# facebookresearch/co-tracker

Hardware: AMD Instinct MI355X
Metric: tracked-point-frames/sec (N*T/s) (higher is better)
Workload: dtype f32 (Linear layers as split-half f16 MFMA x3, f32 accumulate); 1 GPU; 512x512 T=120 N=6400 cotracker3 online-weights sliding window S=16 (BASELINE.json configs[2]); points_per_gpu=6400, frames=120, iters=6, window_len=16, offline=False, precision=f16x3, weights=seeded synthetic (no checkpoints offline)

## Files before the change

co-tracker_amd/csrc/api.hip:

```cpp
#include "ctk_common.h"
#include "ctk_profile.h"
#include "gemm_params.h"
#include "ctk_options.h"
#include <cstdlib>
#include <mutex>
#include <new>

int ctk_launch_corr_volume(const ctk_window_args* a, int n0, int ncount, float* out, long level_stride, int ld,
                           hipStream_t s, bool groups = false);
int ctk_launch_pyramid_split(const float* fmap, long pixels, void* out, int version, hipStream_t s);
int ctk_launch_corr_volume_sh(const ctk_window_args* a, const void* const* fm_sh, int n0, int ncount, void* out,
                              long level_stride_halves, int version, hipStream_t s, bool groups = false);
int ctk_launch_virtual_init(const float* vt, int S, float* dst, int B, hipStream_t s);
int ctk_launch_layernorm2(const float* x, void* y, long R, const float* gamma, const float* beta, float eps, void* y2, float eps2,
                          int out_split, hipStream_t s);
int ctk_launch_heads(const float* tokens, const float* hw, const float* hb, int S, int N, float* delta, float* coords,
                     float* vis, float* conf, hipStream_t s);
int ctk_launch_assemble(const ctk_window_args* a, void* x, int x_split, int ld, int base, hipStream_t s);
int ctk_launch_assemble_batch(const CtkBatchState& st, int B, int S, int N, float scale_x, float scale_y, void* x, int x_split,
                              int ld, int base, hipStream_t s);
int ctk_launch_heads_batch(const float* tokens, const float* hw, const float* hb, const CtkBatchState& st, int B, int S, int N,
                           hipStream_t s);

namespace {

inline size_t align256(size_t x) { return (x + 255) & ~(size_t)255; }

#define CTK_TRY(expr)        \
  do {                       \
    int rc__ = (expr);       \
    if (rc__) return rc__;   \
  } while (0)

class EventRing {
 public:
  int next(hipEvent_t* out) {
    int dev = 0;
    hipError_t rc = hipGetDevice(&dev);
    if (rc != hipSuccess) return (int)rc;
    if (dev < 0 || dev >= kMaxDev) return CTK_E_STATE;
    std::lock_guard<std::mutex> g(m_);
    PerDev& d = d_[dev];
    if (!d.ready) {
      for (int i = 0; i < kN; ++i) {
        rc = hipEventCreateWithFlags(&d.ev[i], hipEventDisableTiming);
        if (rc != hipSuccess) {
          for (int j = 0; j < i; ++j) (void)hipEventDestroy(d.ev[j]);
          return (int)rc;
        }
      }
      d.ready = true;
    }
    *out = d.ev[d.i];
    d.i = (d.i + 1) % kN;
    return CTK_OK;
  }

 private:
  static constexpr int kN = 256, kMaxDev = 64;
  struct PerDev {
    hipEvent_t ev[kN];
    int i = 0;
    bool ready = false;
  };
  std::mutex m_;
  PerDev d_[kMaxDev];
};
EventRing g_events;

int stream_follow(hipStream_t from, hipStream_t to) {
  hipEvent_t e;
  CTK_TRY(g_events.next(&e));
  hipError_t rc = hipEventRecord(e, from);
  if (rc != hipSuccess) return (int)rc;
  rc = hipStreamWaitEvent(to, e, 0);
  return rc == hipSuccess ? CTK_OK : (int)rc;
}

int overlap_mode() { return ctk_opt(CTK_OPT_OVERLAP); }

struct JoinGuard {
  hipStream_t main, aux;
  bool open = false;
  int fork() {
    const int rc = stream_follow(main, aux);
    open = rc == CTK_OK;
    return rc;
  }
  int join() {
    open = false;
    return stream_follow(aux, main);
  }
  ~JoinGuard() {
    if (open) (void)stream_follow(aux, main);
  }
};

struct WRef {
  const float* w;
  const void* p;
};

struct Linear {
  ctk_gemm_args g{};
  Linear(const float* x, long M, WRef W, int N, int K, float* y, const float* bias) {
    g.A = x; g.lda = K; g.M = (int)M; g.W = W.w; g.Wp = W.p; g.ldw = K; g.N = N; g.K = K; g.C = y; g.ldc = N; g.bias = bias;
    g.act = CTK_ACT_NONE; g.batch = 1;
  }
  Linear& act(int a) { g.act = a; return *this; }
  Linear& ldy(long ld) { g.ldc = ld; return *this; }
  Linear& add(const float* resid) { g.resid = resid; return *this; }
  Linear& bias_rows(const float* rows, int period) { g.bias_rows = rows; g.bias_period = period; return *this; }
  Linear& k_valid(int k) { g.k_valid = k; return *this; }
  Linear& batched(int n, long x_bs, long y_bs) { g.batch = n; g.a_bs = x_bs; g.c_bs = y_bs; return *this; }
  Linear& sh(bool in, bool out) { g.a_split = in; g.c_split = out; return *this; }
  int run(hipStream_t s) {
    if (g.resid) g.ldr = g.ldc;
    if (g.a_split) { g.lda *= 2; g.a_bs *= 2; }
    if (g.c_split) { g.ldc *= 2; g.c_bs *= 2; }
    return ctk_gemm(&g, s);
  }
};

bool split_mode(const ctk_model_weights* w) { return w->in_p != nullptr; }
bool folded(const ctk_model_weights* w) { return !w->corr_fc2_w && !w->corr_fc2_p; }

struct UfWs {
  float* tokens;
  float* xn;
  float* xn2;
  float* qkv;
  float* att;
  float* hid;
  float* partial;
  size_t bytes;
};

int v2p_splits(int N) {
  int s = (N + 1023) / 1024;
  if (s < 1) s = 1;
  if (s > 32) s = 32;
  return s;
}

UfWs carve_uf(int S, int N, void* base, int B = 1) {
  const size_t R = (size_t)B * (N + CTK_VIRT) * S;
  UfWs w;
  char* p = static_cast<char*>(base);
  size_t off = 0;
  auto take = [&](size_t nfloat) {
    float* r = reinterpret_cast<float*>(p + off);
    off += align256(nfloat * sizeof(float));
    return r;
  };
  w.tokens = take(R * CTK_HID);
  w.xn = take(R * CTK_HID);
  w.xn2 = take((size_t)B * N * S * CTK_HID);
  w.qkv = take(R * 3 * CTK_HID);
  w.att = take(R * CTK_HID);
  w.hid = take(R * CTK_MLP);
  w.partial = take((size_t)v2p_splits(N) * B * S * CTK_HEADS * CTK_VIRT * (CTK_HEAD_DIM + 2));
  w.bytes = off;
  return w;
}

int attn(const float* q, long q_ld, long q_bs, long q_is, const float* k, const float* v, long kv_ld, long kv_bs,
         long kv_is, float* out, long o_bs, long o_is, int nbatch, int n1, int n2, int splits, float* partial,
         hipStream_t s, bool o_split, const uint8_t* key_mask = nullptr, const uint8_t* query_mask = nullptr,
         const ctk_attn_batch2* b2 = nullptr) {
  ctk_attn_args a;
  a.key_mask = key_mask; a.query_mask = query_mask;
  a.q = q; a.q_ld = q_ld; a.q_bs = q_bs; a.q_is = q_is;
  a.k = k; a.v = v; a.kv_ld = kv_ld; a.kv_bs = kv_bs; a.kv_is = kv_is;
  a.out = out; a.o_ld = o_split ? 2 * CTK_HID : CTK_HID; a.o_bs = o_bs; a.o_is = o_is; a.o_split = o_split;
  a.nbatch = nbatch; a.n1 = n1; a.n2 = n2; a.splits = splits; a.partial = partial;
  return ctk_attention_ex(&a, b2, s);
}

int mlp_block(const UfWs& ws, long r0, long R, const ctk_block_weights& b, hipStream_t s, bool sp) {
  float* tok = ws.tokens + r0 * CTK_HID;
  float* xn = ws.xn + r0 * CTK_HID;
  float* hid = ws.hid + r0 * CTK_MLP;
  CTK_TRY(ctk_layernorm(tok, xn, R, nullptr, nullptr, 1e-6f, sp, s));
  CTK_TRY(Linear(xn, R, {b.w1, b.w1_p}, CTK_MLP, CTK_HID, hid, b.b1).act(CTK_ACT_GELU_TANH).sh(sp, sp).run(s));
  CTK_TRY(Linear(hid, R, {b.w2, b.w2_p}, CTK_HID, CTK_MLP, tok, b.b2).add(tok).sh(sp, false).run(s));
  return CTK_OK;
}

struct FormerRef {
  int depth;
  const ctk_block_weights* time_blocks;
  const ctk_block_weights* virtual2point;
  const ctk_block_weights* virtual_self;
  const ctk_block_weights* point2virtual;
  const float* virtual_tokens;
  const uint8_t* point_mask;
  bool split;
  hipStream_t aux;
  bool space_attn = true;
  int B = 1;
};

FormerRef former_of(const ctk_model_weights* w) {
  return FormerRef{CTK_DEPTH, w->time_blocks, w->virtual2point, w->virtual_self, w->point2virtual, w->virtual_tokens, nullptr,
                   w->in_p != nullptr, nullptr};
}

int run_transformer(int S, int N, const FormerRef& fr, const UfWs& ws, hipStream_t s) {
  const FormerRef* w = &fr;
  const bool sp = fr.split;
  const int B = fr.B;
  const long P = (long)B * N * S;
  const long V = (long)B * CTK_VIRT * S;
  const long PS = (long)N * S, VS = (long)CTK_VIRT * S;
  const bool joint = B > 1;
  if (joint && fr.point_mask) return CTK_E_STATE;
  const ctk_attn_batch2 v2p_b{S, 0, VS, PS, VS, 0, 0};
  const ctk_attn_batch2 vself_b{S, 0, VS, VS, VS, 0, 0};
  const ctk_attn_batch2 p2v_b{S, 0, PS, VS, PS, 0, 0};
  const long R = P + V;
  const long QL = 3 * CTK_HID;
  struct Rows { float *tok, *xn, *att, *q, *k, *v; };
  auto rows_from = [&](long r) {
    return Rows{ws.tokens + r * CTK_HID, ws.xn + r * CTK_HID, ws.att + r * CTK_HID, ws.qkv + r * QL, ws.qkv + r * QL + CTK_HID, ws.qkv + r * QL + 2 * CTK_HID};
  };
  const Rows pt = rows_from(0), vt = rows_from(P);
  auto to_q = [&](const ctk_block_weights& b, const float* xn, long rows, const Rows& q, hipStream_t st) {
    return Linear(xn, rows, {b.wq, b.wq_p}, CTK_HID, CTK_HID, q.q, b.bq).ldy(QL).sh(sp, false).run(st);
  };
  auto to_kv = [&](const ctk_block_weights& b, const Rows& kv, long rows) {
    return Linear(kv.xn, rows, {b.wkv, b.wkv_p}, 2 * CTK_HID, CTK_HID, kv.k, b.bkv).ldy(QL).sh(sp, false).run(s);
  };
  auto to_out = [&](const ctk_block_weights& b, const Rows& q, long rows) {
    return Linear(q.att, rows, {b.wo, b.wo_p}, CTK_HID, CTK_HID, q.tok, b.bo).add(q.tok).sh(sp, false).run(s);
  };
  CTK_TRY(ctk_launch_virtual_init(w->virtual_tokens, S, vt.tok, B, s));

  for (int i = 0; i < fr.depth; ++i) {
    {
      const ctk_block_weights& b = w->time_blocks[i];
      CTK_TRY(ctk_layernorm(pt.tok, pt.xn, R, nullptr, nullptr, 1e-6f, sp, s));
      CTK_TRY(to_q(b, pt.xn, R, pt, s));
      CTK_TRY(to_kv(b, pt, R));
      CTK_TRY(attn(pt.q, QL, S, 1, pt.k, pt.v, QL, S, 1, pt.att, S, 1, B * (N + CTK_VIRT), S, S, 1, nullptr, s, sp));
      CTK_TRY(to_out(b, pt, R));
      CTK_TRY(mlp_block(ws, 0, R, b, s, sp));
    }
    if (!fr.space_attn) continue;
    const bool side_q = fr.aux != nullptr && (overlap_mode() & 2) != 0;
    JoinGuard side{s, fr.aux};
    if (side_q) {
      CTK_TRY(side.fork());
      CTK_TRY(ctk_layernorm(pt.tok, ws.xn2, P, nullptr, nullptr, 1e-6f, sp, fr.aux));
      CTK_TRY(to_q(w->point2virtual[i], ws.xn2, P, pt, fr.aux));
    }
    {
      const ctk_block_weights& b = w->virtual2point[i];
      CTK_TRY(ctk_layernorm(vt.tok, vt.xn, V, nullptr, nullptr, 1e-6f, sp, s));
      if (!side_q) CTK_TRY(ctk_launch_layernorm2(pt.tok, pt.xn, P, b.ctx_gamma, b.ctx_beta, 1e-5f, ws.xn2, 1e-6f, sp, s));
      else CTK_TRY(ctk_layernorm(pt.tok, pt.xn, P, b.ctx_gamma, b.ctx_beta, 1e-5f, sp, s));
      CTK_TRY(to_q(b, vt.xn, V, vt, s));
      CTK_TRY(to_kv(b, pt, P));
      CTK_TRY(attn(vt.q, QL, 1, S, pt.k, pt.v, QL, 1, S, vt.att, 1, S, B * S, CTK_VIRT, N,
                   v2p_splits(N), ws.partial, s, sp, fr.point_mask, nullptr, joint ? &v2p_b : nullptr));
      CTK_TRY(to_out(b, vt, V));
      CTK_TRY(mlp_block(ws, P, V, b, s, sp));
    }
    {
      const ctk_block_weights& b = w->virtual_self[i];
      CTK_TRY(ctk_layernorm(vt.tok, vt.xn, V, nullptr, nullptr, 1e-6f, sp, s));
      CTK_TRY(to_q(b, vt.xn, V, vt, s));
      CTK_TRY(to_kv(b, vt, V));
      CTK_TRY(attn(vt.q, QL, 1, S, vt.k, vt.v, QL, 1, S, vt.att, 1, S, B * S,
                   CTK_VIRT, CTK_VIRT, 1, nullptr, s, sp, nullptr, nullptr, joint ? &vself_b : nullptr));
      CTK_TRY(to_out(b, vt, V));
      CTK_TRY(mlp_block(ws, P, V, b, s, sp));
    }
    {
      const ctk_block_weights& b = w->point2virtual[i];
      CTK_TRY(ctk_layernorm(vt.tok, vt.xn, V, b.ctx_gamma, b.ctx_beta, 1e-5f, sp, s));
      if (!side_q) CTK_TRY(to_q(b, ws.xn2, P, pt, s));
      else CTK_TRY(side.join());
      CTK_TRY(to_kv(b, vt, V));
      CTK_TRY(attn(pt.q, QL, 1, S, vt.k, vt.v, QL, 1, S, pt.att, 1, S, B * S, N, CTK_VIRT, 1, nullptr, s, sp,
                   nullptr, fr.point_mask, joint ? &p2v_b : nullptr));
      CTK_TRY(to_out(b, pt, P));
      CTK_TRY(mlp_block(ws, 0, P, b, s, sp));
    }
  }
  return CTK_OK;
}

int check_former(const FormerRef& fr) {
  auto check_block = [&](const ctk_block_weights& b, bool cross) {
    if (!b.bq || !b.bkv || !b.bo || !b.b1 || !b.b2) return CTK_E_NULL;
    if ((!b.wq && !b.wq_p) || (!b.wkv && !b.wkv_p) || (!b.wo && !b.wo_p) || (!b.w1 && !b.w1_p) || (!b.w2 && !b.w2_p)) return CTK_E_NULL;
    if (cross && (!b.ctx_gamma || !b.ctx_beta)) return CTK_E_NULL;
    const bool all_p = b.wq_p && b.wkv_p && b.wo_p && b.w1_p && b.w2_p, any_p = b.wq_p || b.wkv_p || b.wo_p || b.w1_p || b.w2_p;
    return (fr.split ? !all_p : any_p) ? CTK_E_NULL : CTK_OK;
  };
  for (int i = 0; i < fr.depth; ++i) {
    CTK_TRY(check_block(fr.time_blocks[i], false));
    CTK_TRY(check_block(fr.virtual2point[i], true));
    CTK_TRY(check_block(fr.virtual_self[i], false));
    CTK_TRY(check_block(fr.point2virtual[i], true));
  }
  return CTK_OK;
}

int check_weights(const ctk_model_weights* w, bool window = false) {
  if (!w) return CTK_E_NULL;
  if ((!w->in_w && !w->in_p) || !w->in_bias_t || !w->virtual_tokens || !w->head_w || !w->head_b) return CTK_E_NULL;
  if (folded(w)) {
    if (!window || (!w->corr_fc1_w && !w->corr_fc1_p) || !w->corr_fc1_b) return CTK_E_NULL;
    if (split_mode(w) != (w->corr_fc1_p != nullptr)) return CTK_E_NULL;
  } else if (split_mode(w) != (w->corr_fc1_p && w->corr_fc2_p)) {
    return CTK_E_NULL;
  }
  return check_former(former_of(w));
}

int input_projection(int S, int N, const float* x, bool x_split, const ctk_model_weights* w, const UfWs& ws, hipStream_t s,
                     bool fold = false) {
  return Linear(x, N * S, {w->in_w, w->in_p}, CTK_HID, fold ? CTK_XF_LD : CTK_X_LD, ws.tokens, nullptr)
      .bias_rows(w->in_bias_t, S).k_valid(fold ? CTK_XF_DIM : CTK_X_DIM).sh(x_split, false).run(s);
}

struct CorrWs {
  float* vol;
  float* h1;
  void* fm_sh[CTK_MAX_BATCH][CTK_LEVELS];
  size_t bytes;
  int chunk;
  int corr_version;
};

int corr_chunk_points(const ctk_window_args* a, int B = 1) {
  const long all = (long)B * a->N;
  long c = a->points_per_chunk > 0 ? a->points_per_chunk : all;
  if (c > all) c = all;
  return (int)c;
}

CorrWs carve_corr(const ctk_window_args* a, void* base, int B = 1, bool shared = false, bool fold = false) {
  CorrWs w;
  w.corr_version = ctk_opt(CTK_OPT_CORR_VERSION);
  w.chunk = corr_chunk_points(a, B);
  const size_t rows = (size_t)w.chunk * a->S;
  char* p = static_cast<char*>(base);
  size_t off = 0;
  w.vol = reinterpret_cast<float*>(p + off);
  off += align256(rows * CTK_LEVELS * CTK_CORR_LD * sizeof(float));
  w.h1 = fold ? nullptr : reinterpret_cast<float*>(p + off);
  if (!fold) off += align256(rows * CTK_LEVELS * CTK_HID * sizeof(float));
  for (int b = 0; b < B; ++b)
    for (int l = 0; l < CTK_LEVELS; ++l) {
      if (shared && b > 0) {
        w.fm_sh[b][l] = w.fm_sh[0][l];
        continue;
      }
      w.fm_sh[b][l] = p + off;
      off += align256((size_t)a->S * (a->H[l] > 0 ? a->H[l] : 0) * (a->W[l] > 0 ? a->W[l] : 0) * CTK_C * sizeof(float));
    }
  w.bytes = off;
  return w;
}

int prepare_pyramid_sh(const ctk_window_args* videos, const CorrWs& ws, hipStream_t s, int B = 1) {
  for (int b = 0; b < B; ++b) {
    const ctk_window_args* a = videos + b;
    for (int l = 0; l < CTK_LEVELS; ++l) {
      if (!a->fmaps[l]) return CTK_E_NULL;
      if (a->H[l] <= 0 || a->W[l] <= 0) return CTK_E_SHAPE;
      CTK_TRY(ctk_launch_pyramid_split(a->fmaps[l], (long)a->S * a->H[l] * a->W[l], ws.fm_sh[b][l], ws.corr_version, s));
    }
  }
  return CTK_OK;
}

int run_corr_embed(const ctk_window_args* videos, int B, const ctk_model_weights* w, float* x, bool x_split, const CorrWs& ws,
                   hipStream_t s, bool shared = false, bool fold = false) {
  const ctk_window_args* a = videos;
  const bool sp = split_mode(w);
  if (x_split && !sp) return CTK_E_SHAPE;
  if ((!w->corr_fc1_w && !w->corr_fc1_p) || !w->corr_fc1_b) return CTK_E_NULL;
  if (fold != folded(w) || (!fold && !w->corr_fc2_b)) return CTK_E_NULL;
  hipStream_t aux = B == 1 ? static_cast<hipStream_t>(a->aux_stream) : nullptr;
  const bool pipelined = sp && aux != nullptr && (overlap_mode() & 1) != 0;
  const int NT = B * a->N;
  for (int n0 = 0; n0 < NT; n0 += ws.chunk) {
    const int cnt = (NT - n0 < ws.chunk) ? NT - n0 : ws.chunk;
    const int pieces = pipelined ? ((cnt >= 4096) ? 4 : (cnt >= 1024 ? 2 : 1)) : 1;
    const int per = (cnt + pieces - 1) / pieces;
    JoinGuard pipe{s, aux};
    for (int j = 0; j < pieces; ++j) {
      const int p0 = j * per;
      const int pc = (cnt - p0 < per) ? cnt - p0 : per;
      if (pc <= 0) break;
      const long rows = (long)pc * a->S;
      float* vol = ws.vol + (size_t)p0 * a->S * CTK_LEVELS * CTK_CORR_LD;
      float* h1 = fold ? nullptr : ws.h1 + (size_t)p0 * a->S * CTK_LEVELS * CTK_HID;
      hipStream_t gs = s;
      const int g0 = n0 + p0;
      if (shared && B > 1) {
        if (sp) CTK_TRY(ctk_launch_corr_volume_sh(a, ws.fm_sh[0], g0, pc, vol, rows * CTK_CORR_LD * 2, ws.corr_version, s, true));
        else CTK_TRY(ctk_launch_corr_volume(a, g0, pc, vol, rows * CTK_CORR_LD, CTK_CORR_LD, s, true));
      } else {
        for (int b = g0 / a->N; b < B && b * a->N < g0 + pc; ++b) {
          const int lo = g0 > b * a->N ? g0 : b * a->N;
          const int hi = g0 + pc < (b + 1) * a->N ? g0 + pc : (b + 1) * a->N;
          const int m0 = lo - b * a->N, mc = hi - lo;
          float* vb = vol + (size_t)(lo - g0) * a->S * CTK_CORR_LD;
          if (sp) CTK_TRY(ctk_launch_corr_volume_sh(videos + b, ws.fm_sh[b], m0, mc, vb, rows * CTK_CORR_LD * 2, ws.corr_version, s));
          else CTK_TRY(ctk_launch_corr_volume(videos + b, m0, mc, vb, rows * CTK_CORR_LD, CTK_CORR_LD, s));
        }
      }
      if (pipelined && pieces > 1) {
// ... 453 lines not shown
```

co-tracker_amd/csrc/attention.hip:

```cpp
#include "ctk_common.h"
#include "ctk_options.h"
#include "ctk_profile.h"
#include "gemm_params.h"
#include <cstdlib>

namespace {

constexpr int HD = CTK_HEAD_DIM;
constexpr int KC = 16;
constexpr int MAXB = 8;
constexpr int BPAD = 4;
constexpr float NEG_MAX = -3.402823466e+38f;

struct AttnP {
  const float* q; long q_ld, q_bs, q_is;
  const float* k; const float* v; long kv_ld, kv_bs, kv_is;
  float* out; long o_ld, o_bs, o_is;
  int nbatch, n1, n2;
  int splits, keys_per_split;
  float* partial;
  int o_split;
  int bpw;
  int qtiles;
  float scale;
// ... 820 lines not shown
    }
    if (!more) break;
    job = next;
  }
}

constexpr int TR_LD = 3 * CTK_HID;
constexpr int TR_PITCH = TR_LD + VT_PITCH;
constexpr int TR_CHUNKS = TR_LD / 4;
constexpr int TR_LOADS = 32 * TR_CHUNKS / 512;
static_assert(TR_PITCH % 64 == VT_PITCH && (TR_PITCH * 4) % 16 == 0 && 32 * TR_CHUNKS == 512 * TR_LOADS && TR_CHUNKS % 8 == 0, "pair block layout");
static_assert(16 * TR_CHUNKS == 512 * (TR_LOADS / 2), "a track is a whole number of workgroup loads");
static_assert(32 * TR_PITCH * 4 <= 160 * 1024, "one pair per CU");
constexpr int TR_MIN_ROUNDS = 8;

__global__ __launch_bounds__(512, 1) void attention_time_rows_kernel(AttnP p, int npairs) {
  __shared__ __attribute__((aligned(16))) float blk[32 * TR_PITCH];
  const int tid = threadIdx.x, head = tid >> 6, lane = tid & 63, r32 = lane & 31, half = lane >> 5;
  const int vd0 = r32, vd1 = min(32 + r32, HD - 1);
  const int rb = r32 >> 4, ri = r32 & 15;
  int pair = blockIdx.x;
  if (pair >= npairs) return;
  unsigned char* oimg = reinterpret_cast<unsigned char*>(blk + head * HD);
  const float* qrow = blk + r32 * TR_PITCH + head * HD + half * 8;
  const float* vcol = blk + 2 * CTK_HID + head * HD;

  f32x4 raw[TR_LOADS];
  auto load = [&](const int pr) {
    const float* src = p.q + (long)pr * (32 * TR_LD) + tid * 4;
    const int second = (2 * pr + 1 < p.nbatch) ? (TR_LOADS / 2) * 512 * 4 : 0;
#pragma unroll
    for (int i = 0; i < TR_LOADS / 2; ++i) {
      raw[i] = __builtin_nontemporal_load(reinterpret_cast<const f32x4*>(src + i * 512 * 4));
      raw[i + TR_LOADS / 2] = __builtin_nontemporal_load(reinterpret_cast<const f32x4*>(src + i * 512 * 4 + second));
    }
  };

  load(pair);
  while (true) {
    const int b0 = 2 * pair;
    {
#pragma unroll
      for (int i = 0; i < TR_LOADS / 2; ++i) {
        const int c = 512 * i + tid, row = c / TR_CHUNKS, cc = c - row * TR_CHUNKS;
        float* dst = blk + row * TR_PITCH + cc * 4;
        *reinterpret_cast<f32x4*>(dst) = raw[i];
        *reinterpret_cast<f32x4*>(dst + 16 * TR_PITCH) = raw[i + TR_LOADS / 2];
      }
    }
    const int next = pair + (int)gridDim.x;
    const bool more = next < npairs;
    if (more) load(next);
    __syncthreads();

    f16x8 qh[3], ql[3], kh[3], kl[3], vh[2][2], vl[2][2];
    {
      f32x4 f[6];
#pragma unroll
      for (int j = 0; j < 3; ++j) {
        f[2 * j] = *reinterpret_cast<const f32x4*>(qrow + 16 * j);
        f[2 * j + 1] = *reinterpret_cast<const f32x4*>(qrow + 16 * j + 4);
      }
#pragma unroll
      for (int j = 0; j < 3; ++j) ctk_split8(f[2 * j] * p.scale2, f[2 * j + 1] * p.scale2, qh[j], ql[j]);
#pragma unroll
      for (int j = 0; j < 3; ++j) {
        f[2 * j] = *reinterpret_cast<const f32x4*>(qrow + CTK_HID + 16 * j);
        f[2 * j + 1] = *reinterpret_cast<const f32x4*>(qrow + CTK_HID + 16 * j + 4);
      }
#pragma unroll
      for (int j = 0; j < 3; ++j) ctk_split8(f[2 * j], f[2 * j + 1], kh[j], kl[j]);
    }
    {
      float v0[16], v1[16];
#pragma unroll
      for (int s = 0; s < 2; ++s)
#pragma unroll
        for (int e = 0; e < 8; ++e) {
          const int slot = 16 * s + 8 * (e >> 2) + 4 * half + (e & 3);
          v0[8 * s + e] = vcol[slot * TR_PITCH + vd0];
          v1[8 * s + e] = vcol[slot * TR_PITCH + vd1];
        }
#pragma unroll
      for (int s = 0; s < 2; ++s) {
        ctk_split8(f32x4{v0[8 * s], v0[8 * s + 1], v0[8 * s + 2], v0[8 * s + 3]}, f32x4{v0[8 * s + 4], v0[8 * s + 5], v0[8 * s + 6], v0[8 * s + 7]},
                   vh[0][s], vl[0][s]);
        ctk_split8(f32x4{v1[8 * s], v1[8 * s + 1], v1[8 * s + 2], v1[8 * s + 3]}, f32x4{v1[8 * s + 4], v1[8 * s + 5], v1[8 * s + 6], v1[8 * s + 7]},
                   vh[1][s], vl[1][s]);
      }
    }

    const bool qvalid = b0 + rb < p.nbatch;
    f32x16 sacc;
#pragma unroll
    for (int e = 0; e < 16; ++e) sacc[e] = 0.0f;
#pragma unroll
    for (int j = 0; j < 3; ++j) sacc = ctk_mma3(kh[j], kl[j], qh[j], ql[j], sacc);
    float tmax = -INFINITY;
#pragma unroll
    for (int e = 0; e < 16; ++e) {
      const int slot = 8 * (e >> 2) + 4 * half + (e & 3);
      const bool ok = ((slot >> 4) == rb) && (b0 + (slot >> 4) < p.nbatch);
      sacc[e] = ok ? sacc[e] : -INFINITY;
      tmax = fmaxf(tmax, sacc[e]);
    }
    tmax = fmaxf(tmax, __shfl_xor(tmax, 32, 64));
    const float mnew = (tmax == -INFINITY) ? 0.0f : tmax;
    float l = 0.0f;
#pragma unroll
    for (int e = 0; e < 16; ++e) {
      const float pv = __builtin_amdgcn_exp2f(sacc[e] - mnew);
      l += pv;
      sacc[e] = pv * PSCALE;
    }
    f32x16 oacc[2];
#pragma unroll
    for (int dt = 0; dt < 2; ++dt)
#pragma unroll
      for (int e = 0; e < 16; ++e) oacc[dt][e] = 0.0f;
#pragma unroll
    for (int s = 0; s < 2; ++s) {
      f16x8 ph, pl;
      ctk_split8(f32x4{sacc[8 * s], sacc[8 * s + 1], sacc[8 * s + 2], sacc[8 * s + 3]},
                 f32x4{sacc[8 * s + 4], sacc[8 * s + 5], sacc[8 * s + 6], sacc[8 * s + 7]}, ph, pl);
      oacc[0] = ctk_mma3(vh[0][s], vl[0][s], ph, pl, oacc[0]);
      oacc[1] = ctk_mma3(vh[1][s], vl[1][s], ph, pl, oacc[1]);
    }
    l += __shfl_xor(l, 32, 64);
    const float inv = 1.0f / (l * PSCALE);
    if (p.o_split) {
      attn_store_sh_head<TR_PITCH * 4>(oacc, inv, oimg, lane, head, [&](int row) -> _Float16* {
        const int ob = b0 + (row >> 4), oi = row & 15;
        return ob < p.nbatch ? reinterpret_cast<_Float16*>(p.out) + ((long)ob * p.o_bs + (long)oi * p.o_is) * p.o_ld : nullptr;
      });
    } else if (qvalid) {
      const long orow = ((long)(b0 + rb) * p.o_bs + (long)ri * p.o_is) * p.o_ld;
#pragma unroll
      for (int dt = 0; dt < 2; ++dt)
#pragma unroll
        for (int q = 0; q < 4; ++q) {
          const int d = dt * 32 + q * 8 + half * 4;
          if (d < HD) {
            const f32x4 t = {oacc[dt][4 * q] * inv, oacc[dt][4 * q + 1] * inv, oacc[dt][4 * q + 2] * inv, oacc[dt][4 * q + 3] * inv};
            *reinterpret_cast<f32x4*>(p.out + orow + head * HD + d) = t;
          }
        }
    }
    if (!more) break;
    pair = next;
    __syncthreads();
  }
}

__global__ void attention_merge_kernel(AttnP p) {
  const long i = (long)blockIdx.x * blockDim.x + threadIdx.x;
  const long total = (long)p.nbatch * CTK_HEADS * p.n1 * HD;
  if (i >= total) return;
  const int d = i % HD;
  long r = i / HD;
  const int qi = r % p.n1; r /= p.n1;
  const int head = r % CTK_HEADS;
  const int b = r / CTK_HEADS;
  const long stride = (long)p.nbatch * CTK_HEADS * p.n1 * (HD + 2);
  const float* base = p.partial + (((long)b * CTK_HEADS + head) * p.n1 + qi) * (HD + 2);
  float m = -INFINITY;
  for (int s = 0; s < p.splits; ++s) m = fmaxf(m, base[s * stride]);
  float l = 0.0f, a = 0.0f;
  for (int s = 0; s < p.splits; ++s) {
    const float w = p.log2m ? __builtin_amdgcn_exp2f(base[s * stride] - m) : expf(base[s * stride] - m);
    l += w * base[s * stride + 1];
    a += w * base[s * stride + 2 + d];
  }
  const float o = a / l;
  const long orow = batch_row(b, p.binner, p.o_bs, p.o_obs) + qi * p.o_is;
  if (p.o_split) {
    _Float16* oh = reinterpret_cast<_Float16*>(p.out) + orow * p.o_ld + ctk_sh_col(head * HD + d);
    const _Float16 hi = (_Float16)o;
    oh[0] = hi;
    oh[32] = (_Float16)(o - (float)hi);
  } else {
    p.out[orow * p.o_ld + head * HD + d] = o;
  }
}

int attn_backend() { return ctk_opt(CTK_OPT_ATTENTION_VALU); }

int attn_num_cus() {
  static const int n = [] {
    int dev = 0, cu = 0;
    if (hipGetDevice(&dev) != hipSuccess || hipDeviceGetAttribute(&cu, hipDeviceAttributeMultiprocessorCount, dev) != hipSuccess || cu <= 0) cu = 256;
    return cu;
  }();
  return n;
}

}

extern "C" int ctk_attention(const ctk_attn_args* a, void* stream) { return ctk_attention_ex(a, nullptr, stream); }

extern "C" int ctk_attention_ex(const ctk_attn_args* a, const ctk_attn_batch2* b2, void* stream) {
  if (!a || !a->q || !a->k || !a->v || !a->out) return CTK_E_NULL;
  if (a->nbatch <= 0 || a->n1 <= 0 || a->n2 <= 0) return CTK_E_SHAPE;
  const bool two_level = b2 != nullptr && b2->inner > 0;
  if (two_level && (a->nbatch % b2->inner)) return CTK_E_SHAPE;
  if ((a->q_ld % 4) || (a->kv_ld % 4) || (a->o_ld % 4)) return CTK_E_ALIGN;
  if (!ctk_aligned16(a->q) || !ctk_aligned16(a->k) || !ctk_aligned16(a->v) || !ctk_aligned16(a->out)) return CTK_E_ALIGN;
  AttnP p;
  p.q = a->q; p.q_ld = a->q_ld; p.q_bs = a->q_bs; p.q_is = a->q_is;
  p.k = a->k; p.v = a->v; p.kv_ld = a->kv_ld; p.kv_bs = a->kv_bs; p.kv_is = a->kv_is;
  p.out = static_cast<float*>(a->out); p.o_ld = a->o_ld; p.o_bs = a->o_bs; p.o_is = a->o_is;
  p.o_split = a->o_split;
  if (p.o_split && (a->o_ld % 64)) return CTK_E_ALIGN;
  p.nbatch = a->nbatch; p.n1 = a->n1; p.n2 = a->n2;
  p.splits = a->splits > 1 ? a->splits : 1;
  if (p.splits > 1 && !a->partial) return CTK_E_NULL;
  p.partial = a->partial;
  p.kmask = a->key_mask;
  p.qmask = a->query_mask;
  p.binner = two_level ? b2->inner : a->nbatch;
  p.q_obs = two_level ? b2->q_os : 0; p.kv_obs = two_level ? b2->kv_os : 0; p.o_obs = two_level ? b2->o_os : 0;
  p.km_obs = two_level ? b2->key_mask_os : 0; p.qm_obs = two_level ? b2->query_mask_os : 0;
  p.scale = 0.14433756729740643f;
  p.scale2 = 0.14433756729740643f * 1.4426950408889634f;
  p.log2m = 0;
  hipStream_t s = static_cast<hipStream_t>(stream);
  const double flops = 4.0 * a->nbatch * (double)a->n1 * a->n2 * CTK_HID;
  const double bytes = 4.0 * a->nbatch * ((double)a->n1 * 2 + (double)a->n2 * 2) * CTK_HID;
  const bool mfma = attn_backend() == 0;

  if (mfma && a->n2 == CTK_VIRT) {
    p.splits = 1;
    p.keys_per_split = a->n2;
    p.bpw = 1;
    p.qtiles = 1;
    CtkProfScope ps(a->n1 > CTK_VIRT ? "attention_p2v" : "attention_vself", flops, bytes, s);
    const unsigned gx = (unsigned)((a->n1 + 128 * QT_PER_WG - 1) / (128 * QT_PER_WG));
    hipLaunchKernelGGL(attention_kv64_kernel, dim3(gx, CTK_HEADS, (unsigned)a->nbatch), dim3(256), 0, s, p);
    CTK_HIP_CHECK_LAUNCH();
    return CTK_OK;
  }
  if (mfma && a->n1 == CTK_VIRT && a->n2 > CTK_VIRT) {
    p.keys_per_split = ((a->n2 + p.splits - 1) / p.splits + 31) / 32 * 32;
    p.splits = (a->n2 + p.keys_per_split - 1) / p.keys_per_split;
    p.bpw = 1;
    p.qtiles = 1;
    p.log2m = 1;
    CtkProfScope ps("attention_v2p", flops, bytes, s);
    hipLaunchKernelGGL(attention_q64_kernel, dim3((unsigned)p.splits, CTK_HEADS, (unsigned)a->nbatch), dim3(256), 0, s, p);
    CTK_HIP_CHECK_LAUNCH();
    if (p.splits > 1) {
      const long total = (long)p.nbatch * CTK_HEADS * p.n1 * HD;
      hipLaunchKernelGGL(attention_merge_kernel, dim3((unsigned)((total + 255) / 256)), dim3(256), 0, s, p);
      CTK_HIP_CHECK_LAUNCH();
    }
    return CTK_OK;
  }

  if (mfma && a->n1 == a->n2 && p.splits == 1 && !two_level) {
    p.keys_per_split = a->n2;
    p.bpw = a->n1 <= 16 ? 2 : 1;
    p.qtiles = p.bpw == 2 ? 1 : (a->n1 + 31) / 32;
    const long njobs = (long)((a->nbatch + p.bpw - 1) / p.bpw) * p.qtiles;
    CtkProfScope ps(a->q_is == 1 ? "attention_time" : "attention_vself", flops, bytes, s);
    const int tmode = ctk_opt(CTK_OPT_ATTENTION_TIME_PERSISTENT);
    const bool persistent = tmode != 0;
    const int cus = attn_num_cus();
    const bool pair_block = a->n1 == 16 && a->k == a->q + CTK_HID && a->v == a->q + 2 * CTK_HID && a->q_ld == TR_LD && a->kv_ld == TR_LD &&
                            a->q_is == 1 && a->kv_is == 1 && a->q_bs == a->n1 && a->kv_bs == a->n1;
    const bool rows_kernel = pair_block && (tmode == 3 || (tmode == 1 && njobs >= (long)TR_MIN_ROUNDS * cus));
    if (p.bpw == 2 && !p.kmask && !p.qmask && rows_kernel) {
      hipLaunchKernelGGL(attention_time_rows_kernel, dim3((unsigned)(njobs < cus ? njobs : cus)), dim3(512), 0, s, p, (int)njobs);
    } else if (p.bpw == 2 && !p.kmask && !p.qmask && persistent) {
      const long total = njobs * CTK_HEADS;
      const unsigned blocks = (unsigned)((total + 3) / 4 < 512 ? (total + 3) / 4 : 512);
      hipLaunchKernelGGL(attention_time16_kernel, dim3(blocks), dim3(256), 0, s, p, total);
    } else if (p.bpw == 2) hipLaunchKernelGGL(attention_self_kernel<2>, dim3((unsigned)((njobs + 3) / 4), CTK_HEADS), dim3(256), 0, s, p);
    else hipLaunchKernelGGL(attention_self_kernel<1>, dim3((unsigned)((njobs + 3) / 4), CTK_HEADS), dim3(256), 0, s, p);
    CTK_HIP_CHECK_LAUNCH();
    return CTK_OK;
  }

  p.keys_per_split = ((a->n2 + p.splits - 1) / p.splits + KC - 1) / KC * KC;
  p.splits = (a->n2 + p.keys_per_split - 1) / p.keys_per_split;
  unsigned gx;
  if (a->n1 >= 64) {
    p.bpw = 1;
    p.qtiles = (a->n1 + 63) / 64;
    gx = (unsigned)(p.qtiles * a->nbatch);
  } else {
    p.bpw = 64 / a->n1;
    if (p.bpw > MAXB) p.bpw = MAXB;
    p.qtiles = 1;
    gx = (unsigned)((a->nbatch + p.bpw - 1) / p.bpw);
  }
  const char* pname = p.splits > 1 ? "attention_v2p" : (a->n1 > CTK_VIRT && a->n2 == CTK_VIRT) ? "attention_p2v"
                      : (a->n1 == CTK_VIRT && a->n2 == CTK_VIRT && a->q_is != 1) ? "attention_vself" : "attention_time";
  CtkProfScope ps(pname, flops, bytes, s);
  const size_t lds_bytes = (size_t)2 * p.bpw * (KC * HD + BPAD) * sizeof(float);
  hipLaunchKernelGGL(attention_kernel, dim3(gx, CTK_HEADS, (unsigned)p.splits), dim3(64), lds_bytes, s, p);
  CTK_HIP_CHECK_LAUNCH();
  if (p.splits > 1) {
    const long total = (long)p.nbatch * CTK_HEADS * p.n1 * HD;
    hipLaunchKernelGGL(attention_merge_kernel, dim3((unsigned)((total + 255) / 256)), dim3(256), 0, s, p);
    CTK_HIP_CHECK_LAUNCH();
  }
  return CTK_OK;
}
```

Measured before the change: 650,100 tracked-point-frames/s.

## Add row-blocked virtual-to-point attention kernel sharing K/V tiles across heads

Adds a new virtual-to-point attention kernel in which each workgroup processes four heads, one per wave. The waves cooperatively stage contiguous K|V row segments into shared memory with register prefetch of the next tile, instead of each head gathering its own keys. For large point counts the split count is now chosen from CU count divided by frames, and the partial-workspace sizing is changed to the maximum possible split count. The aim is coalesced K/V reads and better occupancy for the N=6400 key case, at the cost of extra LDS traffic, barriers and more merge partials.

```diff
diff --git a/co-tracker_amd/csrc/api.hip b/co-tracker_amd/csrc/api.hip
--- a/co-tracker_amd/csrc/api.hip
+++ b/co-tracker_amd/csrc/api.hip
@@ -14,6 +14,8 @@
 int ctk_launch_virtual_init(const float* vt, int S, float* dst, int B, hipStream_t s);
 int ctk_launch_layernorm2(const float* x, void* y, long R, const float* gamma, const float* beta, float eps, void* y2, float eps2,
                           int out_split, hipStream_t s);
+bool ctk_attn_v2p_rows_chosen(int n2);
+int ctk_attn_v2p_rows_splits(int frames, int n2);
 int ctk_launch_heads(const float* tokens, const float* hw, const float* hb, int S, int N, float* delta, float* coords,
                      float* vis, float* conf, hipStream_t s);
 int ctk_launch_assemble(const ctk_window_args* a, void* x, int x_split, int ld, int base, hipStream_t s);
@@ -136,11 +138,18 @@
   size_t bytes;
 };
 
-int v2p_splits(int N) {
+int v2p_splits(int N, int frames, bool masked) {
+  if (!masked && ctk_attn_v2p_rows_chosen(N)) return ctk_attn_v2p_rows_splits(frames, N);
   int s = (N + 1023) / 1024;
   if (s < 1) s = 1;
   if (s > 32) s = 32;
   return s;
+}
+
+int v2p_splits_max(int N) {
+  const int tiles = (N + 31) / 32, wave = (N + 1023) / 1024;
+  const int s = tiles > wave ? tiles : wave;
+  return s > 32 ? 32 : s < 1 ? 1 : s;
 }
 
 UfWs carve_uf(int S, int N, void* base, int B = 1) {
@@ -159,7 +168,7 @@
   w.qkv = take(R * 3 * CTK_HID);
   w.att = take(R * CTK_HID);
   w.hid = take(R * CTK_MLP);
-  w.partial = take((size_t)v2p_splits(N) * B * S * CTK_HEADS * CTK_VIRT * (CTK_HEAD_DIM + 2));
+  w.partial = take((size_t)v2p_splits_max(N) * B * S * CTK_HEADS * CTK_VIRT * (CTK_HEAD_DIM + 2));
   w.bytes = off;
   return w;
 }
@@ -262,7 +271,7 @@
       CTK_TRY(to_q(b, vt.xn, V, vt, s));
       CTK_TRY(to_kv(b, pt, P));
       CTK_TRY(attn(vt.q, QL, 1, S, pt.k, pt.v, QL, 1, S, vt.att, 1, S, B * S, CTK_VIRT, N,
-                   v2p_splits(N), ws.partial, s, sp, fr.point_mask, nullptr, joint ? &v2p_b : nullptr));
+                   v2p_splits(N, B * S, fr.point_mask != nullptr), ws.partial, s, sp, fr.point_mask, nullptr, joint ? &v2p_b : nullptr));
       CTK_TRY(to_out(b, vt, V));
       CTK_TRY(mlp_block(ws, P, V, b, s, sp));
     }
diff --git a/co-tracker_amd/csrc/attention.hip b/co-tracker_amd/csrc/attention.hip
--- a/co-tracker_amd/csrc/attention.hip
+++ b/co-tracker_amd/csrc/attention.hip
@@ -996,6 +996,219 @@
   }
 }
 
+constexpr int QR_ROW = 2 * CTK_HID;
+constexpr int QR_HEADS = 4;
+constexpr int QR_SEG = QR_HEADS * HD;
+constexpr int QR_PITCH = 2 * QR_SEG + VT_PITCH;
+constexpr int QR_CH = 2 * QR_SEG / 4;
+constexpr int QR_KG = 192 / QR_CH;
+constexpr int QR_MIN_KEYS = 4000;
+static_assert(QR_PITCH % 64 == VT_PITCH && (QR_PITCH * 4) % 16 == 0 && QR_KG * QR_CH == 192 && 4 * QR_KG * QR_HEADS == 32 &&
+              (QR_SEG * 4) % 128 == 0 && CTK_HEADS % QR_HEADS == 0, "k | v block layout: whole lines, 3 wave loads per group of keys");
+static_assert(QR_HEADS * CTK_VIRT * (HD + 2) <= 32 * QR_PITCH && (CTK_VIRT * (HD + 2)) % 4 == 0, "the partial images fit the block image");
+static_assert((CTK_HEADS / QR_HEADS) * 32 * QR_PITCH * 4 <= 160 * 1024, "eight waves per CU");
+
+__global__ __launch_bounds__(64 * QR_HEADS, 2) void attention_q64_rows_kernel(AttnP p) {
+  __shared__ __attribute__((aligned(16))) float blk[32 * QR_PITCH];
+  const int tid = threadIdx.x, wave = __builtin_amdgcn_readfirstlane(tid >> 6), lane = tid & 63, r32 = lane & 31, half = lane >> 5;
+  const int split = blockIdx.x, hg = blockIdx.y, b = blockIdx.z;
+  const int head = hg * QR_HEADS + wave;
+  const long kvb = batch_row(b, p.binner, p.kv_bs, p.kv_obs);
+  const long qb = batch_row(b, p.binner, p.q_bs, p.q_obs), ob = batch_row(b, p.binner, p.o_bs, p.o_obs);
+
+  f16x8 qh[2][3], ql[2][3];
+#pragma unroll
+  for (int qt = 0; qt < 2; ++qt) {
+    const float* qp = p.q + (qb + (long)(qt * 32 + r32) * p.q_is) * p.q_ld + head * HD + half * 8;
+#pragma unroll
+    for (int j = 0; j < 3; ++j) {
+      const f32x4 a = *reinterpret_cast<const f32x4*>(qp + 16 * j) * p.scale2;
+      const f32x4 c = *reinterpret_cast<const f32x4*>(qp + 16 * j + 4) * p.scale2;
+      ctk_split8(a, c, qh[qt][j], ql[qt][j]);
+    }
+  }
+  const int kbeg = split * p.keys_per_split;
+  const int kend = min(p.n2, kbeg + p.keys_per_split);
+  const int ntiles = (kend - kbeg + 31) >> 5;
+  const float* kvsrc = p.k + kvb * p.kv_ld + hg * QR_SEG;
+  const long kstride = p.kv_is * p.kv_ld;
+  const int vd0 = r32, vd1 = min(32 + r32, HD - 1);
+  const float* krow = blk + r32 * QR_PITCH + wave * HD + half * 8;
+  const float* vcol = blk + QR_SEG + wave * HD;
+  int lsel[3], lcol[3];
+#pragma unroll
+  for (int t = 0; t < 3; ++t) {
+    const int c = 64 * t + lane;
+    lsel[t] = c / QR_CH;
+    lcol[t] = 4 * (c - QR_CH * lsel[t]);
+  }
+
+  f32x4 raw[12];
+  auto load = [&](const int tile) {
+    const int k0 = kbeg + tile * 32 + 4 * QR_KG * wave;
+#pragma unroll
+    for (int r = 0; r < 4; ++r)
+#pragma unroll
+      for (int t = 0; t < 3; ++t) {
+        const float* src = kvsrc + (long)min(k0 + QR_KG * r + lsel[t], kend - 1) * kstride + (lcol[t] < QR_SEG ? lcol[t] : lcol[t] - QR_SEG + CTK_HID);
+        raw[3 * r + t] = *reinterpret_cast<const f32x4*>(src);
+      }
+  };
+
+  float m[2] = {-INFINITY, -INFINITY}, l[2] = {0.0f, 0.0f};
+  f32x16 oacc[2][2];
+#pragma unroll
+  for (int dt = 0; dt < 2; ++dt)
+#pragma unroll
+    for (int qt = 0; qt < 2; ++qt)
+#pragma unroll
+      for (int e = 0; e < 16; ++e) oacc[dt][qt][e] = 0.0f;
+
+  load(0);
+  for (int tile = 0; tile < ntiles; ++tile) {
+    const int k0 = kbeg + tile * 32;
+#pragma unroll
+    for (int r = 0; r < 4; ++r)
+#pragma unroll
+      for (int t = 0; t < 3; ++t) *reinterpret_cast<f32x4*>(blk + (4 * QR_KG * wave + QR_KG * r + lsel[t]) * QR_PITCH + lcol[t]) = raw[3 * r + t];
+    if (tile + 1 < ntiles) load(tile + 1);
+    __syncthreads();
+
+    f16x8 kh[3], kl[3];
+    {
+      f32x4 f[6];
+#pragma unroll
+      for (int j = 0; j < 3; ++j) {
+        f[2 * j] = *reinterpret_cast<const f32x4*>(krow + 16 * j);
+        f[2 * j + 1] = *reinterpret_cast<const f32x4*>(krow + 16 * j + 4);
+      }
+#pragma unroll
+      for (int j = 0; j < 3; ++j) ctk_split8(f[2 * j], f[2 * j + 1], kh[j], kl[j]);
+    }
+    f16x8 ph[2][2], pl[2][2];
+#pragma unroll
+    for (int qt = 0; qt < 2; ++qt) {
+      f32x16 sacc;
+#pragma unroll
+      for (int e = 0; e < 16; ++e) sacc[e] = 0.0f;
+#pragma unroll
+      for (int j = 0; j < 3; ++j) sacc = ctk_mma3(kh[j], kl[j], qh[qt][j], ql[qt][j], sacc);
+      if (k0 + 32 > kend) {
+#pragma unroll
+        for (int e = 0; e < 16; ++e)
+          if (k0 + 8 * (e >> 2) + 4 * half + (e & 3) >= kend) sacc[e] = -INFINITY;
+      }
+      float tmax = -INFINITY;
+#pragma unroll
+      for (int e = 0; e < 16; ++e) tmax = fmaxf(tmax, sacc[e]);
+      tmax = fmaxf(tmax, __shfl_xor(tmax, 32, 64));
+      const float mnew = fmaxf(m[qt], tmax);
+      const float alpha = __builtin_amdgcn_exp2f(m[qt] - mnew);
+      m[qt] = mnew;
+      float psum = 0.0f;
+#pragma unroll
+      for (int e = 0; e < 16; ++e) {
+        const float pv = __builtin_amdgcn_exp2f(sacc[e] - mnew);
+        psum += pv;
+        sacc[e] = pv * PSCALE;
+      }
+      l[qt] = l[qt] * alpha + psum;
+#pragma unroll
+      for (int e = 0; e < 16; ++e) {
+        oacc[0][qt][e] *= alpha;
+        oacc[1][qt][e] *= alpha;
+      }
+#pragma unroll
+      for (int s = 0; s < 2; ++s)
+        ctk_split8(f32x4{sacc[8 * s], sacc[8 * s + 1], sacc[8 * s + 2], sacc[8 * s + 3]},
+                   f32x4{sacc[8 * s + 4], sacc[8 * s + 5], sacc[8 * s + 6], sacc[8 * s + 7]}, ph[qt][s], pl[qt][s]);
+    }
+    __builtin_amdgcn_sched_barrier(0);
+    f16x8 vh[2][2], vl[2][2];
+    {
+      float vraw[2][16];
+#pragma unroll
+      for (int s = 0; s < 2; ++s)
+#pragma unroll
+        for (int e = 0; e < 8; ++e) {
+          const int key = 16 * s + 8 * (e >> 2) + 4 * half + (e & 3);
+          vraw[0][s * 8 + e] = vcol[key * QR_PITCH + vd0];
+          vraw[1][s * 8 + e] = vcol[key * QR_PITCH + vd1];
+        }
+      __syncthreads();
+#pragma unroll
+      for (int dt = 0; dt < 2; ++dt)
+#pragma unroll
+        for (int s = 0; s < 2; ++s) {
+          const f32x4 a = {vraw[dt][s * 8], vraw[dt][s * 8 + 1], vraw[dt][s * 8 + 2], vraw[dt][s * 8 + 3]};
+          const f32x4 c = {vraw[dt][s * 8 + 4], vraw[dt][s * 8 + 5], vraw[dt][s * 8 + 6], vraw[dt][s * 8 + 7]};
+          ctk_split8(a, c, vh[dt][s], vl[dt][s]);
+        }
+    }
+#pragma unroll
+    for (int s = 0; s < 2; ++s)
+#pragma unroll
+      for (int dt = 0; dt < 2; ++dt)
+#pragma unroll
+        for (int qt = 0; qt < 2; ++qt) oacc[dt][qt] = ctk_mma3(vh[dt][s], vl[dt][s], ph[qt][s], pl[qt][s], oacc[dt][qt]);
+  }
+
+  if (p.splits == 1) {
+#pragma unroll
+    for (int qt = 0; qt < 2; ++qt) {
+      const float inv = 1.0f / ((l[qt] + __shfl_xor(l[qt], 32, 64)) * PSCALE);
+      const long orow = (ob + (long)(qt * 32 + r32) * p.o_is) * p.o_ld;
+#pragma unroll
+      for (int dt = 0; dt < 2; ++dt)
+#pragma unroll
+        for (int q = 0; q < 4; ++q) {
+          const int d = dt * 32 + q * 8 + half * 4;
+          if (d < HD) {
+            const f32x4 t = {oacc[dt][qt][4 * q] * inv, oacc[dt][qt][4 * q + 1] * inv, oacc[dt][qt][4 * q + 2] * inv, oacc[dt][qt][4 * q + 3] * inv};
+            if (p.o_split) {
+              f16x4 hi, lo;
+              ctk_split4(t, hi, lo);
+              _Float16* dst = reinterpret_cast<_Float16*>(p.out) + orow + ctk_sh_col(head * HD + d);
+              *reinterpret_cast<f16x4*>(dst) = hi;
+              *reinterpret_cast<f16x4*>(dst + 32) = lo;
+            } else {
+              *reinterpret_cast<f32x4*>(p.out + orow + head * HD + d) = t;
+            }
+          }
+        }
+    }
+  } else {
+    float* img = blk + wave * (CTK_VIRT * (HD + 2));
+#pragma unroll
+    for (int qt = 0; qt < 2; ++qt) {
+      const float lsum = l[qt] + __shfl_xor(l[qt], 32, 64);
+      float* rr = img + (qt * 32 + r32) * (HD + 2);
+      if (half == 0) {
+        rr[0] = m[qt];
+        rr[1] = lsum;
+      }
+#pragma unroll
+      for (int dt = 0; dt < 2; ++dt)
+#pragma unroll
+        for (int q = 0; q < 4; ++q) {
+          const int d = dt * 32 + q * 8 + half * 4;
+          if (d < HD) {
+#pragma unroll
+            for (int e = 0; e < 4; ++e) rr[2 + d + e] = oacc[dt][qt][4 * q + e] * (1.0f / PSCALE);
+          }
+        }
+    }
+    __builtin_amdgcn_wave_barrier();
+    float* pp = p.partial + (((long)split * p.nbatch + b) * CTK_HEADS + head) * (CTK_VIRT * (HD + 2));
+    constexpr int CHUNKS = CTK_VIRT * (HD + 2) / 4;
+#pragma unroll
+    for (int i = 0; i < (CHUNKS + 63) / 64; ++i) {
+      const int c = 64 * i + lane;
+      if (c < CHUNKS) *reinterpret_cast<f32x4*>(pp + 4 * c) = *reinterpret_cast<const f32x4*>(img + 4 * c);
+    }
+  }
+}
+
 __global__ void attention_merge_kernel(AttnP p) {
   const long i = (long)blockIdx.x * blockDim.x + threadIdx.x;
   const long total = (long)p.nbatch * CTK_HEADS * p.n1 * HD;
@@ -1038,6 +1251,18 @@
   return n;
 }
 
+}
+
+bool ctk_attn_v2p_rows_chosen(int n2) {
+  return attn_backend() == 0 && (n2 >= QR_MIN_KEYS || ctk_opt(CTK_OPT_ATTENTION_TIME_PERSISTENT) == 3);
+}
+
+int ctk_attn_v2p_rows_splits(int frames, int n2) {
+  int s = (attn_num_cus() + frames - 1) / (frames > 0 ? frames : 1);
+  const int tiles = (n2 + 31) / 32;
+  if (s > tiles) s = tiles;
+  if (s > 32) s = 32;
+  return s < 1 ? 1 : s;
 }
 
 extern "C" int ctk_attention(const ctk_attn_args* a, void* stream) { return ctk_attention_ex(a, nullptr, stream); }
@@ -1083,14 +1308,18 @@
     CTK_HIP_CHECK_LAUNCH();
     return CTK_OK;
   }
-  if (mfma && a->n1 == CTK_VIRT && a->n2 > CTK_VIRT) {
+  const bool kv_rows = mfma && a->n1 == CTK_VIRT && a->n2 != CTK_VIRT && !a->key_mask && !a->query_mask && a->v == a->k + CTK_HID &&
+                       a->kv_ld == QR_ROW + CTK_HID && (p.splits == 1 || ctk_aligned16(a->partial)) && a->nbatch <= 65535 &&
+                       ctk_attn_v2p_rows_chosen(a->n2);
+  if (mfma && a->n1 == CTK_VIRT && (a->n2 > CTK_VIRT || kv_rows)) {
     p.keys_per_split = ((a->n2 + p.splits - 1) / p.splits + 31) / 32 * 32;
     p.splits = (a->n2 + p.keys_per_split - 1) / p.keys_per_split;
     p.bpw = 1;
     p.qtiles = 1;
     p.log2m = 1;
     CtkProfScope ps("attention_v2p", flops, bytes, s);
-    hipLaunchKernelGGL(attention_q64_kernel, dim3((unsigned)p.splits, CTK_HEADS, (unsigned)a->nbatch), dim3(256), 0, s, p);
+    if (kv_rows) hipLaunchKernelGGL(attention_q64_rows_kernel, dim3((unsigned)p.splits, CTK_HEADS / QR_HEADS, (unsigned)a->nbatch), dim3(64 * QR_HEADS), 0, s, p);
+    else hipLaunchKernelGGL(attention_q64_kernel, dim3((unsigned)p.splits, CTK_HEADS, (unsigned)a->nbatch), dim3(256), 0, s, p);
     CTK_HIP_CHECK_LAUNCH();
     if (p.splits > 1) {
       const long total = (long)p.nbatch * CTK_HEADS * p.n1 * HD;
```

After: 653,600 tracked-point-frames/s, median of 6. Within noise of the previous version (+0.5%).
